# HorizonRobotics/HoloAgent

Measured on AMD Instinct MI355X. Metric: HMSG frames/sec (one scene per GPU: map A1-A2, fusion A3-A5, merge A6, pooling A7, floors A8, rooms by the device watershed N1, room clouds, room embeddings and View nodes A9, objects with the view <-> object test A10 and graph assembly A11, nothing handed in -- plus 1000 coarse-to-fine retrieval qu, higher is better.
Workload: dtype f64 geometry / f32 features

## Files before the change

holoagent_amd/csrc/hmsg_dbscan.h:

```cpp
#pragma once
#include "hmsg_common.h"

#include <vector>

struct PoolSeg {
    long long row_base;
    long long bit_base;
    int n;
    int nw;
    long long tile_base;
    int nt;
    int pad;
};

#define GRAM_T 128

void pool_launch_gram_f32(hipStream_t s, const float* Xn, int D, const PoolSeg* d_ps, int K, long long tiles, float eps, unsigned* adj,
                          unsigned* ncount);
void pool_launch_seg_rows(hipStream_t s, const PoolSeg* d_ps, int K, int maxn, int* seg_of_row);
void pool_cluster(hipStream_t s, const PoolSeg* d_ps, long long R, int minpts, const unsigned* adj, const unsigned* ncount,
                  const int* seg_of_row, int* label, int* seg_first, int* d_changed, int* flabel, unsigned* csize, unsigned* cfirst,
                  unsigned long long* best, DbgLaps* laps = nullptr);
void pool_launch_mean_f32(hipStream_t s, const float* X, int D, const PoolSeg* d_ps, int K, const int* flabel, const unsigned* csize,
                          const unsigned* cfirst, const unsigned long long* best, float* out);

void rn_denoise(hipStream_t s, const void* X, bool f64, int D, const std::vector<long long>& off, double eps, int min_samples, void* out,
                int* n_in_cluster);
void rn_choose(hipStream_t s, const void* rows, bool f64, long long K, int D, const float* T, int n_types, int* d_type);
void rn_vote(hipStream_t s, const int* d_view_type, const std::vector<long long>& voff, int n_types, int* type_of_room );
void rn_gather_rows_f32(hipStream_t s, const float* src, const std::vector<int>& rows, int D, float* dst);
```

holoagent_amd/csrc/hmsg_map.hip:

```cpp
#include "hmsg_common.h"

#include <atomic>

#include <algorithm>


__global__ void k_scan_lookback(const unsigned* __restrict__ in, unsigned* __restrict__ out, size_t n,
                                unsigned long long* __restrict__ state, unsigned epoch) {
    __shared__ unsigned wsum[4];
    __shared__ unsigned s_prefix;
    const int tid = threadIdx.x, lane = tid & 63, w = tid >> 6;
    const long long tile = blockIdx.x;
    const size_t base = ((size_t)tile * 256 + tid) * 4;
    unsigned v[4];
    unsigned t = 0;
    for (int i = 0; i < 4; ++i) {
        v[i] = base + i < n ? in[base + i] : 0u;
        t += v[i];
    }
    unsigned incl = t;
    for (int o = 1; o < 64; o <<= 1) {
        unsigned u = __shfl_up(incl, o);
        if (lane >= o) incl += u;
    }
// ... 133 lines not shown
            atomicMax(&out[3 + a], enc_f64(mx[a]));
        }
        atomicAdd(npts, (unsigned long long)c);
    }
}

__global__ void k_mark(const unsigned short* __restrict__ depth, const double* __restrict__ pose, CamK cam, float scale,
                       int H, int W, int F, GridGeom g, unsigned long long* __restrict__ bitmap) {
    const size_t HW = (size_t)H * W;
    const size_t total = HW * F;
    for (size_t c0 = (size_t)blockIdx.x * PIX_CHUNK; c0 < total; c0 += (size_t)gridDim.x * PIX_CHUNK) {
        const PixWalk pw = pix_walk(c0, HW, W);
        const unsigned npix = (unsigned)(total - c0 < (size_t)PIX_CHUNK ? total - c0 : (size_t)PIX_CHUNK);
        const unsigned fl = pix_last_frame(pw, npix);
        for (unsigned ff = pw.f0; ff <= fl; ++ff) {
            const double* const T = pose + (size_t)ff * 16;
            for (unsigned d = threadIdx.x; d < npix; d += blockDim.x) {
                const size_t i = c0 + d;
                int f, x, y;
                pix_at(pw, d, f, x, y);
                double wx, wy, wz;
                if ((unsigned)f != ff || !backproject(depth[i], x, y, cam, scale, T, wx, wy, wz)) continue;
                int ix, iy, iz;
                cell_of(g, wx, wy, wz, ix, iy, iz);
                long long lin = lin_of(g, ix, iy, iz);
                unsigned long long bit = 1ull << (lin & 63);
                unsigned long long* wp = bitmap + (lin >> 6);
                if (!(*wp & bit)) atomicOr(wp, bit);
            }
        }
    }
}

struct VoxAcc {
    unsigned long long* sr;
    unsigned long long* sg;
    unsigned long long* sb;
    unsigned* n;
};

#define RUN_CHUNK 4096
__device__ __forceinline__ unsigned pixel_slot(const unsigned short* __restrict__ depth, const double* __restrict__ T ,
                                               const CamK& cam, float scale, size_t i, int x, int y, const GridGeom& g,
                                               const unsigned long long* __restrict__ bitmap, const unsigned* __restrict__ rank) {
    double wx, wy, wz;
    if (!backproject(depth[i], x, y, cam, scale, T, wx, wy, wz)) return 0xffffffffu;
    int ix, iy, iz;
    cell_of(g, wx, wy, wz, ix, iy, iz);
    const long long lin = lin_of(g, ix, iy, iz);
    const unsigned long long word = bitmap[lin >> 6];
    return rank[lin >> 6] + (unsigned)__popcll(word & ((1ull << (lin & 63)) - 1ull));
}

__global__ void __launch_bounds__(256) k_slots(const unsigned short* __restrict__ depth, const unsigned char* __restrict__ rgb,
                                               const double* __restrict__ pose, CamK cam, float scale, int H, int W, int F,
                                               GridGeom g, const unsigned long long* __restrict__ bitmap,
                                               const unsigned* __restrict__ rank, VoxAcc acc, unsigned* __restrict__ slots,
                                               unsigned* __restrict__ chunk_runs) {
    __shared__ unsigned s_runs;
    if (threadIdx.x == 0) s_runs = 0u;
    __syncthreads();
    const size_t HW = (size_t)H * W;
    const size_t total = HW * F;
    const int lane = threadIdx.x & 63;
    unsigned myruns = 0;
    const PixWalk pw = pix_walk((size_t)blockIdx.x * RUN_CHUNK, HW, W);
    const size_t left = total - (size_t)blockIdx.x * RUN_CHUNK;
    const unsigned fl = pix_last_frame(pw, (unsigned)(left < (size_t)RUN_CHUNK ? left : (size_t)RUN_CHUNK));
    for (int it = 0; it < RUN_CHUNK / 256; ++it) {
        const size_t i = (size_t)blockIdx.x * RUN_CHUNK + (size_t)it * 256 + threadIdx.x;
        const bool in_range = i < total;
        unsigned slot = 0xffffffffu;
        unsigned cr = 0, cg = 0, cb = 0, cn = 0;
        int x = 0;
        if (in_range) {
            int f, y;
            pix_at(pw, (unsigned)it * 256u + threadIdx.x, f, x, y);
            for (unsigned ff = pw.f0; ff <= fl; ++ff)
                if ((unsigned)f == ff) slot = pixel_slot(depth, pose + (size_t)ff * 16, cam, scale, i, x, y, g, bitmap, rank);
            slots[i] = slot;
            if (slot != 0xffffffffu) {
                const unsigned char* c = rgb + i * 3;
                cr = c[0];
                cg = c[1];
                cb = c[2];
                cn = 1;
            }
        }
        const unsigned prev = __shfl_up(slot, 1);
        int flag = (lane == 0 || prev != slot || x == 0) ? 1 : 0;
        const int head = flag;
        for (int d = 1; d < 64; d <<= 1) {
            unsigned tr = __shfl_up(cr, d), tg = __shfl_up(cg, d), tb = __shfl_up(cb, d), tn = __shfl_up(cn, d);
            int tf = __shfl_up(flag, d);
            if (lane >= d && !flag) {
                cr += tr; cg += tg; cb += tb; cn += tn;
                flag = tf;
            }
        }
        const int nhead = __shfl_down(head, 1);
        const bool tail = lane == 63 || nhead != 0;
        if (tail && slot != 0xffffffffu) {
            atomicAdd(&acc.sr[slot], (unsigned long long)cr);
            atomicAdd(&acc.sg[slot], (unsigned long long)cg);
            atomicAdd(&acc.sb[slot], (unsigned long long)cb);
            atomicAdd(&acc.n[slot], cn);
            ++myruns;
        }
    }
    myruns = (unsigned)wave_sum_i32((int)myruns);
    if (lane == 0 && myruns) atomicAdd(&s_runs, myruns);
    __syncthreads();
    if (threadIdx.x == 0) chunk_runs[blockIdx.x] = s_runs;
}

__global__ void __launch_bounds__(256) k_emit_runs(const unsigned* __restrict__ slots, size_t total, int W, size_t HW,
                                                   const unsigned* __restrict__ chunk_base, unsigned* __restrict__ keys,
                                                   unsigned long long* __restrict__ vals) {
    __shared__ unsigned s_w[4];
    __shared__ unsigned s_run;
    if (threadIdx.x == 0) s_run = chunk_base[blockIdx.x];
    __syncthreads();
    const int lane = threadIdx.x & 63, w = threadIdx.x >> 6;
    const PixWalk pw = pix_walk((size_t)blockIdx.x * RUN_CHUNK, HW, W);
    for (int it = 0; it < RUN_CHUNK / 256; ++it) {
        const size_t i = (size_t)blockIdx.x * RUN_CHUNK + (size_t)it * 256 + threadIdx.x;
        const bool in_range = i < total;
        const unsigned slot = in_range ? slots[i] : 0xffffffffu;
        int pf = 0, x = 0, py = 0;
        if (in_range) pix_at(pw, (unsigned)it * 256u + threadIdx.x, pf, x, py);
        const unsigned prev = __shfl_up(slot, 1);
        const bool head = lane == 0 || prev != slot || x == 0;
        const unsigned long long heads = __ballot(head);
        const int nhead = __shfl_down(head ? 1 : 0, 1);
        const bool tail = (lane == 63 || nhead != 0) && slot != 0xffffffffu;
        const unsigned long long tails = __ballot(tail);
        if (lane == 0) s_w[w] = (unsigned)__popcll(tails);
        __syncthreads();
        unsigned base = s_run;
// ... 77 lines not shown
        }
    }
    if (LDS_SUM) {
        if (lane < 3) pts[v * 3 + lane] = __ddiv_rn(sx, (double)cnt[v]);
    } else if (lane == 0) {
        const double n = (double)cnt[v];
        pts[v * 3 + 0] = __ddiv_rn(sx, n);
        pts[v * 3 + 1] = __ddiv_rn(sy, n);
        pts[v * 3 + 2] = __ddiv_rn(sz, n);
    }
}

__global__ void k_slot_cells(const unsigned long long* __restrict__ bitmap, const unsigned* __restrict__ rank,
                             GridGeom g, int* __restrict__ cell ) {
    long long w = (long long)blockIdx.x * blockDim.x + threadIdx.x;
    if (w >= g.nwords) return;
    unsigned long long bits = bitmap[w];
    unsigned s = rank[w];
    while (bits) {
        int b = __ffsll(bits) - 1;
        bits &= bits - 1;
        long long lin = w * 64 + b;
        int iz = (int)(lin % g.nzp);
        long long r = lin / g.nzp;
        int iy = (int)(r % g.ny);
        int ix = (int)(r / g.ny);
        cell[(size_t)s * 3 + 0] = ix;
        cell[(size_t)s * 3 + 1] = iy;
        cell[(size_t)s * 3 + 2] = iz;
        ++s;
    }
}

__global__ void k_finalize(VoxAcc acc, long long V, double* __restrict__ cols) {
    long long s = (long long)blockIdx.x * blockDim.x + threadIdx.x;
    if (s >= V) return;
    double n = (double)acc.n[s];
    cols[s * 3 + 0] = ((double)acc.sr[s] / 255.0) / n;
    cols[s * 3 + 1] = ((double)acc.sg[s] / 255.0) / n;
    cols[s * 3 + 2] = ((double)acc.sb[s] / 255.0) / n;
}

__device__ __forceinline__ unsigned long long bits_range(int lo, int hi) {
    if (hi < lo) return 0ull;
    unsigned long long m = (hi >= 63) ? ~0ull : ((1ull << (hi + 1)) - 1ull);
    return m & ~((1ull << lo) - 1ull);
}

__global__ void k_outlier(const double* __restrict__ pts, const int* __restrict__ cell, long long V, GridGeom g,
                          const unsigned long long* __restrict__ bitmap, const unsigned* __restrict__ rank,
                          double radius, int nb_points, unsigned* __restrict__ keep) {
    const int lane = threadIdx.x & 63;
    const long long s = ((long long)blockIdx.x * blockDim.x + threadIdx.x) >> 6;
    if (s >= V) return;
    const double px = pts[s * 3], py = pts[s * 3 + 1], pz = pts[s * 3 + 2];
    const int cx = cell[s * 3], cy = cell[s * 3 + 1];
    const int R = (int)ceil(radius / g.vs) + 1;
    const int side = 2 * R + 1;
    const double r2 = radius * radius;
    const double slack = 1e-7;
    int count = 0;
    for (int c = lane; c < side * side; c += 64) {
        int ix = cx - R + c / side, iy = cy - R + c % side;
        if (ix < 0 || iy < 0 || ix >= g.nx || iy >= g.ny) continue;
        double xlo = g.ox + ix * g.vs, xhi = xlo + g.vs, ylo = g.oy + iy * g.vs, yhi = ylo + g.vs;
        double dxmin = fmax(0.0, fmax(xlo - px, px - xhi)), dxmax = fmax(fabs(px - xlo), fabs(px - xhi));
        double dymin = fmax(0.0, fmax(ylo - py, py - yhi)), dymax = fmax(fabs(py - ylo), fabs(py - yhi));
        dxmin = fmax(0.0, dxmin - slack);
        dymin = fmax(0.0, dymin - slack);
        dxmax += slack;
        dymax += slack;
        double rem_out = r2 - (dxmin * dxmin + dymin * dymin);
        if (rem_out <= 0.0) continue;
// ... 9 lines not shown
            if (hi_ > 0.0) {
                zi0 = (int)ceil((pz - hi_ - g.oz) / g.vs);
                zi1 = (int)floor((pz + hi_ - g.oz) / g.vs) - 1;
                zi0 = zi0 < zo0 ? zo0 : zi0;
                zi1 = zi1 > zo1 ? zo1 : zi1;
            }
        }
        long long colw = ((long long)ix * g.ny + iy) * (g.nzp >> 6);
        for (int w = zo0 >> 6; w <= zo1 >> 6; ++w) {
            unsigned long long word = bitmap[colw + w];
            if (!word) continue;
            int b0 = w * 64;
            unsigned long long outer = word & bits_range(zo0 - b0 < 0 ? 0 : zo0 - b0, zo1 - b0 > 63 ? 63 : zo1 - b0);
            unsigned long long inner = 0ull;
            if (zi1 >= zi0) inner = outer & bits_range(zi0 - b0 < 0 ? 0 : zi0 - b0, zi1 - b0 > 63 ? 63 : zi1 - b0);
            count += __popcll(inner);
            unsigned long long shell = outer & ~inner;
            unsigned base = rank[colw + w];
            while (shell) {
                int b = __ffsll(shell) - 1;
                shell &= shell - 1;
                unsigned q = base + (unsigned)__popcll(word & ((1ull << b) - 1ull));
                double dx = pts[(size_t)q * 3] - px, dy = pts[(size_t)q * 3 + 1] - py, dz = pts[(size_t)q * 3 + 2] - pz;
                double d2 = dx * dx + dy * dy + dz * dz;
                count += d2 < r2 ? 1 : 0;
            }
        }
    }
    count = wave_sum_i32(count);
    if (lane == 0) keep[s] = count > nb_points ? 1u : 0u;
}

__global__ void k_compact(const unsigned* __restrict__ keep, const unsigned* __restrict__ newidx, long long V0,
                          const double* __restrict__ pts0, const double* __restrict__ cols0, const int* __restrict__ cell,
                          GridGeom g, double* __restrict__ pts, double* __restrict__ cols,
                          unsigned long long* __restrict__ bitmap) {
    long long s = (long long)blockIdx.x * blockDim.x + threadIdx.x;
    if (s >= V0) return;
    if (keep[s]) {
        unsigned d = newidx[s];
        for (int a = 0; a < 3; ++a) {
            pts[(size_t)d * 3 + a] = pts0[s * 3 + a];
            cols[(size_t)d * 3 + a] = cols0[s * 3 + a];
        }
    } else {
        long long lin = lin_of(g, cell[s * 3], cell[s * 3 + 1], cell[s * 3 + 2]);
        atomicAnd(&bitmap[lin >> 6], ~(1ull << (lin & 63)));
    }
}

__global__ void k_rm_cells(const unsigned* __restrict__ keep, const unsigned* __restrict__ newidx, long long V0,
                           const int* __restrict__ cell, GridGeom g, int* __restrict__ rmcell,
                           unsigned long long* __restrict__ bitmap_rm) {
    long long s = (long long)blockIdx.x * blockDim.x + threadIdx.x;
    if (s >= V0 || keep[s]) return;
    long long r = s - (long long)newidx[s];
    for (int a = 0; a < 3; ++a) rmcell[r * 3 + a] = cell[s * 3 + a];
    long long lin = lin_of(g, cell[s * 3], cell[s * 3 + 1], cell[s * 3 + 2]);
    atomicOr(&bitmap_rm[lin >> 6], 1ull << (lin & 63));
}

template <typename F>
__device__ __forceinline__ void ring_visit(const GridGeom& g, const unsigned long long* __restrict__ bitmap,
                                           const unsigned* __restrict__ rank, int cx, int cy, int cz, int r, int lane, F&& f) {
    const int side = 2 * r + 1;
    for (int ci = lane; ci < side * side; ci += 64) {
        int dx = ci / side - r, dy = ci % side - r;
        int ix = cx + dx, iy = cy + dy;
        if (ix < 0 || iy < 0 || ix >= g.nx || iy >= g.ny) continue;
        bool rim = (dx == -r || dx == r || dy == -r || dy == r);
        long long colw = ((long long)ix * g.ny + iy) * (g.nzp >> 6);
        for (int part = 0; part < (rim ? 1 : 2); ++part) {
            int z0 = rim ? cz - r : (part == 0 ? cz - r : cz + r);
            int z1 = rim ? cz + r : z0;
            z0 = z0 < 0 ? 0 : z0;
            z1 = z1 >= g.nz ? g.nz - 1 : z1;
            if (!rim && (z0 != z1 || (part == 0 ? cz - r < 0 : cz + r >= g.nz))) continue;
// ... 100 lines not shown
                       (const double*)h->pose.p, h->cam, scale, H, W, F, d_b.p, d_b.p + 6);
    HMSG_CHECK_LAUNCH();
    unsigned long long hb[8];
    HIP_TRY(hipMemcpyAsync(hb, d_b.p, sizeof(hb), hipMemcpyDeviceToHost, s));
    HIP_TRY(hipStreamSynchronize(s));
    HMSG_REQUIRE(hb[6] > 0, HMSG_ERR_INVALID, "no valid depth pixel in any frame");
    double mn[3], mx[3];
    for (int a = 0; a < 3; ++a) {
        mn[a] = dec_f64(hb[a]);
        mx[a] = dec_f64(hb[3 + a]);
    }
    GridGeom g;
    g.vs = c.voxel_size;
    g.ox = mn[0] - g.vs * 0.5;
    g.oy = mn[1] - g.vs * 0.5;
    g.oz = mn[2] - g.vs * 0.5;
    g.nx = (int)floor((mx[0] - g.ox) / g.vs) + 2;
    g.ny = (int)floor((mx[1] - g.oy) / g.vs) + 2;
    g.nz = (int)floor((mx[2] - g.oz) / g.vs) + 2;
    g.nzp = (g.nz + 63) / 64 * 64;
    g.nwords = (long long)g.nx * g.ny * (g.nzp / 64);
    HMSG_REQUIRE(g.nwords < (1ll << 31), HMSG_ERR_UNSUPPORTED, "scene bounding box too large for the dense occupancy bitmap");
    h->grid = g;

    h->bitmap.alloc((size_t)g.nwords);
    h->rank.alloc((size_t)g.nwords);
    h->bitmap.zero(s);
    hipLaunchKernelGGL(k_mark, dim3(nblk), dim3(256), 0, s, (const unsigned short*)h->depth.p, (const double*)h->pose.p,
                       h->cam, scale, H, W, F, g, h->bitmap.p);
    HMSG_CHECK_LAUNCH();
    unsigned long long V0 = hmsg_bitmap_rank(h->bitmap.p, h->rank.p, (size_t)g.nwords, s, h->scan_tmp);
    h->V0 = (long long)V0;

    DevBuf<unsigned long long> srgb;
    DevBuf<unsigned> sn, slots, chunk_runs;
    srgb.alloc(V0 * 3);
    sn.alloc(V0);
    srgb.zero(s);
    sn.zero(s);
    slots.alloc(total);
    const unsigned nchunks = cdiv(total, RUN_CHUNK);
    chunk_runs.alloc((size_t)nchunks + 1);
    VoxAcc acc{srgb.p, srgb.p + V0, srgb.p + 2 * V0, sn.p};
    {
        ProfScope ps(h->prof, s, "k_slots", (double)total * 9.0 + (double)V0 * 28.0);
        hipLaunchKernelGGL(k_slots, dim3(nchunks), dim3(256), 0, s, (const unsigned short*)h->depth.p,
                           (const unsigned char*)h->rgb.p, (const double*)h->pose.p, h->cam, scale, H, W, F, g,
                           (const unsigned long long*)h->bitmap.p, (const unsigned*)h->rank.p, acc, slots.p, chunk_runs.p);
    }
    HMSG_CHECK_LAUNCH();
    unsigned long long nruns = 0;
    hmsg_scan_u32(chunk_runs.p, chunk_runs.p, (size_t)nchunks, s, h->scan_tmp, &nruns);
    SortBufs sb;
    sb.keys.alloc((size_t)std::max<unsigned long long>(nruns, 1));
    sb.vals.alloc((size_t)std::max<unsigned long long>(nruns, 1));
    HMSG_REQUIRE(W < 4096 && H < 4096, HMSG_ERR_UNSUPPORTED, "image sides must be below 4096 pixels");
    hipLaunchKernelGGL(k_emit_runs, dim3(nchunks), dim3(256), 0, s, (const unsigned*)slots.p, total, W, (size_t)H * W,
                       (const unsigned*)chunk_runs.p, sb.keys.p, sb.vals.p);
    HMSG_CHECK_LAUNCH();
    {
        ProfScope ps(h->prof, s, "sort_runs", (double)nruns * 12.0 * 4.0);
        hmsg_sort_pairs(sb, (size_t)nruns, bits_for(V0), s);
    }
    DevBuf<unsigned> run_off;
    run_off.alloc(V0 + 1);
    hmsg_sort_segment_starts(sb.res_keys, (size_t)nruns, run_off.p, (unsigned)V0, s);
    DevBuf<int> cell;
    cell.alloc(V0 * 3);
    hipLaunchKernelGGL(k_slot_cells, dim3(cdiv((size_t)g.nwords, 256)), dim3(256), 0, s,
                       (const unsigned long long*)h->bitmap.p, (const unsigned*)h->rank.p, g, cell.p);
    HMSG_CHECK_LAUNCH();
    DevBuf<double> pts0, cols0;
    pts0.alloc(V0 * 3);
    cols0.alloc(V0 * 3);
    {
        static const bool lds_sum = getenv("HMSG_DEBUG_ACCUM_WAVES") == nullptr;
        ProfScope ps(h->prof, s, "k_accum_ordered", (double)total * 2.0 + (double)nruns * 8.0 + (double)V0 * 32.0);
        hipLaunchKernelGGL(lds_sum ? k_accum_ordered<true> : k_accum_ordered<false>, dim3(cdiv(V0 * 64, 256)), dim3(256), 0, s,
                           (const unsigned short*)h->depth.p, (const double*)h->pose.p, h->cam, scale, W, (size_t)H * W, (long long)V0,
                           (const unsigned*)run_off.p, (const unsigned long long*)sb.res_vals, (const unsigned*)sn.p, pts0.p);
        HMSG_CHECK_LAUNCH();
        if (getenv("HMSG_DEBUG_ACCUM_STATS")) {
            std::vector<unsigned> hc((size_t)V0);
            HIP_TRY(hipMemcpyAsync(hc.data(), sn.p, (size_t)V0 * 4, hipMemcpyDeviceToHost, s));
            HIP_TRY(hipStreamSynchronize(s));
            std::sort(hc.begin(), hc.end());
            double tot = 0;
            for (unsigned c : hc) tot += c;
            fprintf(stderr, "[hmsg map] voxels %lld  runs %llu  pixels %.0f  max %u  median %u  p99 %u\n", (long long)V0, nruns, tot, hc.back(),
                    hc[hc.size() / 2], hc[(size_t)(hc.size() * 0.99)]);
            for (unsigned th : {512u, 2048u, 8192u, 32768u, 131072u}) {
                double px = 0;
                long long nv = 0;
                for (unsigned c : hc)
                    if (c > th) px += c, ++nv;
                fprintf(stderr, "[hmsg map]   more than %6u pixels: %7lld voxels holding %.3f of the pixels\n", th, nv, px / tot);
            }
        }
    }
    hipLaunchKernelGGL(k_finalize, dim3(cdiv(V0, 256)), dim3(256), 0, s, acc, (long long)V0, cols0.p);
    HMSG_CHECK_LAUNCH();

    DevBuf<unsigned> keep, newidx;
    keep.alloc(V0);
    newidx.alloc(V0);
    hipLaunchKernelGGL(k_outlier, dim3(cdiv(V0 * 64, 256)), dim3(256), 0, s, (const double*)pts0.p, (const int*)cell.p,
                       (long long)V0, g, (const unsigned long long*)h->bitmap.p, (const unsigned*)h->rank.p,
                       c.outlier_radius, c.outlier_nb_points, keep.p);
    HMSG_CHECK_LAUNCH();
    unsigned long long V = 0;
    hmsg_scan_u32(keep.p, newidx.p, V0, s, h->scan_tmp, &V);
    h->V = (long long)V;
    h->pts.alloc(V * 3);
    h->cols.alloc(V * 3);
    hipLaunchKernelGGL(k_compact, dim3(cdiv(V0, 256)), dim3(256), 0, s, (const unsigned*)keep.p, (const unsigned*)newidx.p,
                       (long long)V0, (const double*)pts0.p, (const double*)cols0.p, (const int*)cell.p, g, h->pts.p,
                       h->cols.p, h->bitmap.p);
    HMSG_CHECK_LAUNCH();
    unsigned long long V2 = hmsg_bitmap_rank(h->bitmap.p, h->rank.p, (size_t)g.nwords, s, h->scan_tmp);
    HMSG_REQUIRE(V2 == V, HMSG_ERR_INVALID, "internal: filtered bitmap population mismatch");
    const long long VR = (long long)V0 - (long long)V;
    h->have_cand = false;
    if (VR > 0 && V > 0) {
        h->bitmap_rm.alloc((size_t)g.nwords);
        h->rank_rm.alloc((size_t)g.nwords);
        h->bitmap_rm.zero(s);
        DevBuf<int> rmcell, rend;
        DevBuf<double> ub2;
        DevBuf<unsigned> ccnt, cursor;
        rmcell.alloc((size_t)VR * 3);
        rend.alloc((size_t)VR);
        ub2.alloc((size_t)VR);
        ccnt.alloc((size_t)VR + 1);
        cursor.alloc((size_t)VR);
        ccnt.zero(s);
        cursor.zero(s);
        hipLaunchKernelGGL(k_rm_cells, dim3(cdiv(V0, 256)), dim3(256), 0, s, (const unsigned*)keep.p, (const unsigned*)newidx.p,
                           (long long)V0, (const int*)cell.p, g, rmcell.p, h->bitmap_rm.p);
        HMSG_CHECK_LAUNCH();
        unsigned long long nrm = hmsg_bitmap_rank(h->bitmap_rm.p, h->rank_rm.p, (size_t)g.nwords, s, h->scan_tmp);
        HMSG_REQUIRE((long long)nrm == VR, HMSG_ERR_INVALID, "internal: removed-cell bitmap population mismatch");
        h->cand_off.alloc((size_t)VR + 1);
        {
            ProfScope ps(h->prof, s, "k_cand");
            hipLaunchKernelGGL(k_cand, dim3(cdiv((size_t)VR * 64, 256)), dim3(256), 0, s, 0, (const int*)rmcell.p, VR, g,
                               (const unsigned long long*)h->bitmap.p, (const unsigned*)h->rank.p, (const double*)h->pts.p, ub2.p,
                               rend.p, ccnt.p, (const unsigned*)nullptr, (int*)nullptr, (unsigned*)nullptr);
        }
        HMSG_CHECK_LAUNCH();
        unsigned long long ncand = 0;
// ... 13 lines not shown
```

holoagent_amd/csrc/hmsg_pool.hip:

```cpp
#include "hmsg_boundary.h"
#include "hmsg_cloudops.h"
#include "hmsg_nn.h"
#include "hmsg_dbscan.h"

#include <algorithm>
#include <cmath>

typedef float f32x16 __attribute__((ext_vector_type(16)));

__global__ void k_pool_nn(const double* __restrict__ q, long long N, NNIndex I, double max_dist, int* __restrict__ idx,
                          unsigned* __restrict__ valid, TieList ties) {
    long long i = (long long)blockIdx.x * blockDim.x + threadIdx.x;
    if (i >= N) return;
    double d2 = 0;
    int ntie = 0;
    int v = nn_search(I, q[i * 3], q[i * 3 + 1], q[i * 3 + 2], &d2, &ntie);
    if (ntie > 1) tie_push(ties, i, q[i * 3], q[i * 3 + 1], q[i * 3 + 2]);
    idx[i] = v;
    valid[i] = (v >= 0 && __dsqrt_rn(d2) <= max_dist) ? 1u : 0u;
}

__global__ void k_pool_gather(const int* __restrict__ idx, const unsigned* __restrict__ valid, const unsigned* __restrict__ pos,
                              long long N, const float* __restrict__ feats, int D, float* __restrict__ X, float* __restrict__ Xn) {
    const int lane = threadIdx.x & 63;
    const long long i = ((long long)blockIdx.x * blockDim.x + threadIdx.x) >> 6;
    if (i >= N || !valid[i]) return;
    const float* src = feats + (size_t)idx[i] * D;
    float* dx = X + (size_t)pos[i] * D;
    float* dn = Xn + (size_t)pos[i] * D;
    float n2 = 0.f;
    for (int e = lane; e < D; e += 64) {
        float v = src[e];
        if (v != v) v = 0.f;
        else if (v > 3.4028234663852886e38f) v = 3.4028234663852886e38f;
        else if (v < -3.4028234663852886e38f) v = -3.4028234663852886e38f;
        dx[e] = v;
        n2 += v * v;
    }
    float nrm = __fsqrt_rn(wave_sum_f32(n2));
    if (nrm == 0.f) nrm = 1.f;
    for (int e = lane; e < D; e += 64) dn[e] = __fdiv_rn(dx[e], nrm);
}

#define GRAM_SUP 8
__device__ __forceinline__ void gram_tile_of(long long t, int nt, int& ti, int& tj) {
    int I = 0, r0 = 0, hgt = 0;
    for (;;) {
        r0 = I * GRAM_SUP;
        hgt = min(nt, r0 + GRAM_SUP) - r0;
        const long long cnt = (long long)hgt * (nt - r0) - (long long)hgt * (hgt - 1) / 2;
        if (t < cnt) break;
        t -= cnt;
        ++I;
    }
    const long long dcnt = (long long)hgt * (hgt + 1) / 2;
    if (t < dcnt) {
        int r = 0, len = hgt;
        while (t >= len) {
            t -= len;
            --len;
            ++r;
        }
        ti = r0 + r;
        tj = ti + (int)t;
        return;
    }
    t -= dcnt;
    for (int J = I + 1;; ++J) {
        const int w = min(GRAM_SUP, nt - J * GRAM_SUP);
        const long long c = (long long)hgt * w;
        if (t < c) {
            ti = r0 + (int)(t / w);
            tj = J * GRAM_SUP + (int)(t % w);
            return;
// ... 196 lines not shown
        const unsigned* row = adj + sg.bit_base + (size_t)(i - sg.row_base) * sg.nw;
        for (int w = lane; w < sg.nw; w += 64) {
            unsigned bits = row[w];
            while (bits) {
                int b = __ffs(bits) - 1;
                bits &= bits - 1;
                long long j = sg.row_base + (long long)w * 32 + b;
                if (ncount[j] >= (unsigned)minpts) best = label[j] < best ? label[j] : best;
            }
        }
        for (int o = 32; o > 0; o >>= 1) {
            int t = __shfl_xor(best, o);
            best = t < best ? t : best;
        }
        if (best == 0x7fffffff) best = -1;
    }
    if (lane == 0) {
        final_label[i] = best;
        if (best >= 0) {
            atomicAdd(&csize[sg.row_base + best], 1u);
            atomicMin(&cfirst[sg.row_base + best], (unsigned)(i - sg.row_base));
        }
    }
}
__global__ void k_pool_pick(const PoolSeg* __restrict__ segs, const int* __restrict__ seg_of_row, long long N,
                            const unsigned* __restrict__ csize, const unsigned* __restrict__ cfirst,
                            unsigned long long* __restrict__ best) {
    long long i = (long long)blockIdx.x * blockDim.x + threadIdx.x;
    if (i >= N || csize[i] == 0u) return;
    unsigned long long key = ((unsigned long long)csize[i] << 32) | (unsigned long long)(0xffffffffu - cfirst[i]);
    atomicMax(&best[seg_of_row[i]], key);
}
#define POOL_MEAN_AHEAD 16
__global__ void k_pool_mean(const float* __restrict__ X, int D, const PoolSeg* __restrict__ segs, int K,
                            const int* __restrict__ final_label, const unsigned* __restrict__ csize,
                            const unsigned* __restrict__ cfirst, const unsigned long long* __restrict__ best,
                            float* __restrict__ out) {
    const int k = blockIdx.y;
    const int d = blockIdx.x * blockDim.x + threadIdx.x;
    if (d >= D) return;
    const PoolSeg sg = segs[k];
    float* o = out + (size_t)k * D;
    if (sg.n == 0) {
        o[d] = 0.f;
        return;
    }
    int want = -2;
    unsigned long long key = best[k];
    if (key) {
        unsigned first = 0xffffffffu - (unsigned)(key & 0xffffffffull);
        want = final_label[sg.row_base + first];
    }
    float acc = 0.f;
    unsigned cnt = 0;
    const float* const xb = X + (size_t)sg.row_base * D + d;
    const int* const lb = final_label + sg.row_base;
    float cur[POOL_MEAN_AHEAD], nxt[POOL_MEAN_AHEAD];
    int curl[POOL_MEAN_AHEAD], nxtl[POOL_MEAN_AHEAD];
#pragma unroll
    for (int j = 0; j < POOL_MEAN_AHEAD; ++j) {
        const int rr = min(j, sg.n - 1);
        cur[j] = xb[(size_t)rr * D];
        curl[j] = lb[rr];
    }
    for (int r = 0; r < sg.n; r += POOL_MEAN_AHEAD) {
        if (r + POOL_MEAN_AHEAD < sg.n) {
#pragma unroll
            for (int j = 0; j < POOL_MEAN_AHEAD; ++j) {
                const int rr = min(r + POOL_MEAN_AHEAD + j, sg.n - 1);
                nxt[j] = xb[(size_t)rr * D];
                nxtl[j] = lb[rr];
            }
        }
#pragma unroll
        for (int j = 0; j < POOL_MEAN_AHEAD; ++j) {
            if (r + j < sg.n && (want == -2 || curl[j] == want)) {
                acc = __fadd_rn(acc, cur[j]);
                ++cnt;
            }
        }
#pragma unroll
        for (int j = 0; j < POOL_MEAN_AHEAD; ++j) {
            cur[j] = nxt[j];
            curl[j] = nxtl[j];
        }
    }
    o[d] = cnt > 1 ? __fdiv_rn(acc, (float)cnt) : acc;
}

__global__ void k_pool_gather_u32(const unsigned* __restrict__ src, const long long* __restrict__ idx, int n,
                                  unsigned* __restrict__ dst) {
    int t = blockIdx.x * blockDim.x + threadIdx.x;
    if (t < n) dst[t] = src[idx[t]];
}
__global__ void k_seg_rows(const PoolSeg* __restrict__ segs, int* __restrict__ seg_of_row) {
    const PoolSeg sg = segs[blockIdx.y];
    for (int i = blockIdx.x * blockDim.x + threadIdx.x; i < sg.n; i += gridDim.x * blockDim.x) seg_of_row[sg.row_base + i] = blockIdx.y;
}

void pool_cluster(hipStream_t s, const PoolSeg* d_ps, long long R, int minpts, const unsigned* adj, const unsigned* ncount,
                  const int* seg_of_row, int* label, int* seg_first, int* d_changed, int* flabel, unsigned* csize, unsigned* cfirst,
                  unsigned long long* best, DbgLaps* laps) {
    hipLaunchKernelGGL(k_pool_init, dim3(cdiv((size_t)R, 256)), dim3(256), 0, s, ncount, (long long)R,
                       minpts, label, d_ps, seg_of_row, seg_first);
    HMSG_CHECK_LAUNCH();
    DevBuf<unsigned> open_list;
    open_list.alloc((size_t)std::max<long long>(R, 1) + 1);
    const unsigned* d_list = nullptr;
    unsigned n_open = 0;
    static const bool list_wanted = getenv("HMSG_DEBUG_POOL_ALL_ROWS") == nullptr;
    for (int it = 0; it < 100000; ++it) {
        HIP_TRY(hipMemsetAsync(d_changed, 0, 4, s));
        const size_t rows = d_list ? (size_t)n_open : (size_t)R;
        for (int rep = 0; rep < (it == 0 ? 2 : 1) && rows; ++rep) {
            hipLaunchKernelGGL(k_pool_prop, dim3(cdiv(rows * 64, 256)), dim3(256), 0, s, adj,
                               d_ps, seg_of_row, ncount,
                               minpts, (long long)rows, label, d_changed, seg_first, (it == 0 && rep == 0) ? 1 : 0, d_list);
// ... 5 lines not shown
            HIP_TRY(hipMemsetAsync(open_list.p, 0, 4, s));
            hipLaunchKernelGGL(k_pool_list, dim3(cdiv((size_t)R, 256)), dim3(256), 0, s, d_ps, seg_of_row,
                               ncount, minpts, (long long)R, label, seg_first,
                               open_list.p + 1, open_list.p);
            HMSG_CHECK_LAUNCH();
            HIP_TRY(hipMemcpyAsync(&n_open, open_list.p, 4, hipMemcpyDeviceToHost, s));
        }
        int ch = 0;
        HIP_TRY(hipMemcpyAsync(&ch, d_changed, 4, hipMemcpyDeviceToHost, s));
        HIP_TRY(hipStreamSynchronize(s));
        if (it == 0 && list_wanted) d_list = open_list.p + 1;
        if (!ch) break;
    }
    if (laps) laps->lap("label propagation");
    hipLaunchKernelGGL(k_pool_border, dim3(cdiv((size_t)R * 64, 256)), dim3(256), 0, s, adj,
                       d_ps, seg_of_row, ncount, minpts,
                       (long long)R, label, flabel, csize, cfirst);
    hipLaunchKernelGGL(k_pool_pick, dim3(cdiv((size_t)R, 256)), dim3(256), 0, s, d_ps,
                       seg_of_row, (long long)R, csize, cfirst, best);
    HMSG_CHECK_LAUNCH();
}

void pool_launch_gram_f32(hipStream_t s, const float* Xn, int D, const PoolSeg* d_ps, int K, long long tiles, float eps, unsigned* adj,
                          unsigned* ncount) {
    hipLaunchKernelGGL(k_pool_gram, dim3((unsigned)tiles), dim3(256), 0, s, Xn, D, d_ps, K, eps, adj, ncount);
    HMSG_CHECK_LAUNCH();
}
void pool_launch_seg_rows(hipStream_t s, const PoolSeg* d_ps, int K, int maxn, int* seg_of_row) {
    hipLaunchKernelGGL(k_seg_rows, dim3(std::max(1u, std::min(cdiv(maxn, 256), 256u)), K), dim3(256), 0, s, d_ps, seg_of_row);
    HMSG_CHECK_LAUNCH();
}
void pool_launch_mean_f32(hipStream_t s, const float* X, int D, const PoolSeg* d_ps, int K, const int* flabel, const unsigned* csize,
                          const unsigned* cfirst, const unsigned long long* best, float* out) {
    hipLaunchKernelGGL(k_pool_mean, dim3(cdiv(D, 64), K), dim3(64), 0, s, X, D, d_ps, K, flabel, csize, cfirst, best, out);
    HMSG_CHECK_LAUNCH();
}

static void pool_rows(hipStream_t s, DevBuf<unsigned>& scan_tmp, Prof* prof, DbgLaps& laps, const int* idx, const unsigned* valid,
                      long long P, const std::vector<int>& dn, const float* feats, int D, double eps, int minpts, float* out) {
    const int K = (int)dn.size();
    DevBuf<unsigned> pos;
    pos.alloc((size_t)std::max<long long>(P, 1));
    unsigned long long R = 0;
    if (P) hmsg_scan_u32(valid, pos.p, (size_t)P, s, scan_tmp, &R);
    std::vector<long long> pstart(K + 1, 0);
    for (int k = 0; k < K; ++k) pstart[k + 1] = pstart[k] + dn[k];
    std::vector<unsigned> hpos(K + 1, (unsigned)R);
    {
        DevBuf<long long> d_i;
        DevBuf<unsigned> d_o;
        std::vector<long long> q;
        std::vector<int> which;
        for (int k = 0; k < K; ++k)
            if (pstart[k] < P) {
                q.push_back(pstart[k]);
                which.push_back(k);
            }
        if (!q.empty()) {
            std::vector<unsigned> tmp(q.size());
            d_i.alloc(q.size());
            d_o.alloc(q.size());
            HIP_TRY(hipMemcpyAsync(d_i.p, q.data(), q.size() * 8, hipMemcpyHostToDevice, s));
            hipLaunchKernelGGL(k_pool_gather_u32, dim3(cdiv(q.size(), 256)), dim3(256), 0, s, (const unsigned*)pos.p,
                               (const long long*)d_i.p, (int)q.size(), d_o.p);
            HIP_TRY(hipMemcpyAsync(tmp.data(), d_o.p, q.size() * 4, hipMemcpyDeviceToHost, s));
            HIP_TRY(hipStreamSynchronize(s));
            for (size_t t = 0; t < q.size(); ++t) hpos[which[t]] = tmp[t];
        }
        for (int k = K - 1; k >= 0; --k)
            if (pstart[k] >= P) hpos[k] = hpos[k + 1];
    }
    std::vector<PoolSeg> ps(K);
    long long bitw = 0, tiles = 0;
    int maxn = 0;
    for (int k = 0; k < K; ++k) {
        PoolSeg& g = ps[k];
        g.row_base = hpos[k];
        g.n = (int)(hpos[k + 1] - hpos[k]);
        g.nw = (g.n + 31) / 32;
        g.nt = (g.n + GRAM_T - 1) / GRAM_T;
        g.bit_base = bitw;
        g.tile_base = tiles;
        g.pad = 0;
        bitw += (long long)g.n * g.nw;
        tiles += (long long)g.nt * (g.nt + 1) / 2;
        maxn = std::max(maxn, g.n);
    }
    DevBuf<PoolSeg> d_ps;
    d_ps.alloc(K);
    HIP_TRY(hipMemcpyAsync(d_ps.p, ps.data(), (size_t)K * sizeof(PoolSeg), hipMemcpyHostToDevice, s));
    DevBuf<float> X, Xn;
    DevBuf<unsigned> adj, ncount, csize, cfirst;
    DevBuf<int> label, flabel, seg_of_row, d_changed, seg_first;
    DevBuf<unsigned long long> best;
    const size_t Rn = (size_t)std::max<unsigned long long>(R, 1);
    X.alloc(Rn * D);
    Xn.alloc(Rn * D);
    adj.alloc((size_t)std::max<long long>(bitw, 1));
    ncount.alloc(Rn);
    csize.alloc(Rn);
    cfirst.alloc(Rn);
    label.alloc(Rn);
    flabel.alloc(Rn);
    seg_of_row.alloc(Rn);
    d_changed.alloc(1);
    seg_first.alloc((size_t)std::max(K, 1));
    HIP_TRY(hipMemsetAsync(seg_first.p, 0x7f, (size_t)std::max(K, 1) * 4, s));
    best.alloc(K);
    adj.zero(s);
    ncount.zero(s);
    csize.zero(s);
    HIP_TRY(hipMemsetAsync(cfirst.p, 0xff, Rn * 4, s));
    best.zero(s);
    laps.lap("row offsets + buffers");
    if (R) {
        hipLaunchKernelGGL(k_pool_gather, dim3(cdiv((size_t)P * 64, 256)), dim3(256), 0, s, idx,
                           valid, (const unsigned*)pos.p, P, feats, D, X.p, Xn.p);
        hipLaunchKernelGGL(k_seg_rows, dim3(std::max(1u, std::min(cdiv(maxn, 256), 256u)), K), dim3(256), 0, s,
                           (const PoolSeg*)d_ps.p, seg_of_row.p);
        laps.lap("gather + normalise");
        {
            double flop = 0;
            for (auto& g : ps) flop += (double)g.n * ((double)g.n + 1.0) * D;
            ProfScope psc(prof, s, "k_pool_gram", flop);
            hipLaunchKernelGGL(k_pool_gram, dim3((unsigned)tiles), dim3(256), 0, s, (const float*)Xn.p, D, (const PoolSeg*)d_ps.p, K,
                               (float)eps, adj.p, ncount.p);
        }
        laps.lap("k_pool_gram");
        pool_cluster(s, (const PoolSeg*)d_ps.p, (long long)R, minpts, (const unsigned*)adj.p, (const unsigned*)ncount.p,
                     (const int*)seg_of_row.p, label.p, seg_first.p, d_changed.p, flabel.p, csize.p, cfirst.p, best.p, &laps);
    }
    laps.lap("border + pick");
    hmsg_dump("pool_ncount", ncount.p, (size_t)R * 4, s);
    hmsg_dump("pool_flabel", flabel.p, (size_t)R * 4, s);
    hmsg_dump("pool_label", label.p, (size_t)R * 4, s);
    hmsg_dump("pool_segs", d_ps.p, (size_t)K * sizeof(PoolSeg), s);
    hipLaunchKernelGGL(k_pool_mean, dim3(cdiv(D, 64), K), dim3(64), 0, s, (const float*)X.p, D, (const PoolSeg*)d_ps.p, K,
                       (const int*)flabel.p, (const unsigned*)csize.p, (const unsigned*)cfirst.p,
                       (const unsigned long long*)best.p, out);
    HMSG_CHECK_LAUNCH();
    HIP_TRY(hipStreamSynchronize(s));
    laps.lap("k_pool_mean");
}

void hmsg_pool(hmsg_ctx* h) {
    const hmsg_config& c = h->cfg;
    hipStream_t s = h->stream;
    HMSG_REQUIRE(h->merged, HMSG_ERR_INVALID, "hmsg_pool_instances: run hmsg_merge_instances first");
    const int K = (int)h->inst.off.size() - 1;
    const int D = c.feat_dim;
    h->inst_feats.alloc((size_t)std::max(K, 1) * D);
    if (K == 0) {
        h->pooled = true;
        return;
    }
    CloudOps ops;
    ops.s = s;
    DbgLaps laps("pool", s);
    std::vector<SegDesc> segs(K);
    for (int k = 0; k < K; ++k) {
        segs[k].pt_base = h->inst.off[k];
        segs[k].n = (int)(h->inst.off[k + 1] - h->inst.off[k]);
    }
    ops.bounds(h->inst.pts.p, segs);
    DevBuf<double> ds;
    ds.alloc((size_t)std::max<long long>(h->inst.total, 1) * 3);
    std::vector<int> dn;
    const long long P = ops.voxel_down_sample(h->inst.pts.p, segs, c.voxel_size, ds.p, dn);
    laps.lap("voxel_down_sample");
    DevBuf<int> idx;
    DevBuf<unsigned> valid;
    idx.alloc((size_t)std::max<long long>(P, 1));
    valid.alloc((size_t)std::max<long long>(P, 1));
// ... 61 lines not shown
```

Measured before the change: 2639.

## Defer voxel colour sums to kept voxels and gather pooled features by index

Voxel colour accumulation no longer does three 64-bit atomics per run in k_slots. Colours are now computed only for kept voxels after compaction, by walking the sorted run records and reading RGB again. The pooling stage drops the dense X copy of features and stores only a source-row index. The mean kernel then gathers from the original feature table, with nan_to_num applied on the fly and a deeper prefetch of labels and indices. This cuts atomics, buffer traffic and one full feature copy, in exchange for scattered gather reads and a second pass over RGB.

Result: faster. 2683, median of 4 (+1.7%).

```diff
diff --git a/holoagent_amd/csrc/hmsg_dbscan.h b/holoagent_amd/csrc/hmsg_dbscan.h
--- a/holoagent_amd/csrc/hmsg_dbscan.h
+++ b/holoagent_amd/csrc/hmsg_dbscan.h
@@ -23,6 +23,8 @@
                   unsigned long long* best, DbgLaps* laps = nullptr);
 void pool_launch_mean_f32(hipStream_t s, const float* X, int D, const PoolSeg* d_ps, int K, const int* flabel, const unsigned* csize,
                           const unsigned* cfirst, const unsigned long long* best, float* out);
+void pool_launch_mean_gather_f32(hipStream_t s, const float* table, const int* src_row, int D, const PoolSeg* d_ps, int K, const int* flabel,
+                                 const unsigned* csize, const unsigned* cfirst, const unsigned long long* best, float* out);
 
 void rn_denoise(hipStream_t s, const void* X, bool f64, int D, const std::vector<long long>& off, double eps, int min_samples, void* out,
                 int* n_in_cluster);
diff --git a/holoagent_amd/csrc/hmsg_map.hip b/holoagent_amd/csrc/hmsg_map.hip
--- a/holoagent_amd/csrc/hmsg_map.hip
+++ b/holoagent_amd/csrc/hmsg_map.hip
@@ -189,13 +189,6 @@
     }
 }
 
-struct VoxAcc {
-    unsigned long long* sr;
-    unsigned long long* sg;
-    unsigned long long* sb;
-    unsigned* n;
-};
-
 #define RUN_CHUNK 4096
 __device__ __forceinline__ unsigned pixel_slot(const unsigned short* __restrict__ depth, const double* __restrict__ T ,
                                                const CamK& cam, float scale, size_t i, int x, int y, const GridGeom& g,
@@ -209,11 +202,10 @@
     return rank[lin >> 6] + (unsigned)__popcll(word & ((1ull << (lin & 63)) - 1ull));
 }
 
-__global__ void __launch_bounds__(256) k_slots(const unsigned short* __restrict__ depth, const unsigned char* __restrict__ rgb,
-                                               const double* __restrict__ pose, CamK cam, float scale, int H, int W, int F,
+__global__ void __launch_bounds__(256) k_slots(const unsigned short* __restrict__ depth, const double* __restrict__ pose, CamK cam, float scale, int H, int W, int F,
                                                GridGeom g, const unsigned long long* __restrict__ bitmap,
-                                               const unsigned* __restrict__ rank, VoxAcc acc, unsigned* __restrict__ slots,
-                                               unsigned* __restrict__ chunk_runs) {
+                                               const unsigned* __restrict__ rank, unsigned* __restrict__ vox_n,
+                                               unsigned* __restrict__ slots, unsigned* __restrict__ chunk_runs) {
     __shared__ unsigned s_runs;
     if (threadIdx.x == 0) s_runs = 0u;
     __syncthreads();
@@ -228,7 +220,7 @@
         const size_t i = (size_t)blockIdx.x * RUN_CHUNK + (size_t)it * 256 + threadIdx.x;
         const bool in_range = i < total;
         unsigned slot = 0xffffffffu;
-        unsigned cr = 0, cg = 0, cb = 0, cn = 0;
+        unsigned cn = 0;
         int x = 0;
         if (in_range) {
             int f, y;
@@ -236,32 +228,23 @@
             for (unsigned ff = pw.f0; ff <= fl; ++ff)
                 if ((unsigned)f == ff) slot = pixel_slot(depth, pose + (size_t)ff * 16, cam, scale, i, x, y, g, bitmap, rank);
             slots[i] = slot;
-            if (slot != 0xffffffffu) {
-                const unsigned char* c = rgb + i * 3;
-                cr = c[0];
-                cg = c[1];
-                cb = c[2];
-                cn = 1;
-            }
+            if (slot != 0xffffffffu) cn = 1;
         }
         const unsigned prev = __shfl_up(slot, 1);
         int flag = (lane == 0 || prev != slot || x == 0) ? 1 : 0;
         const int head = flag;
         for (int d = 1; d < 64; d <<= 1) {
-            unsigned tr = __shfl_up(cr, d), tg = __shfl_up(cg, d), tb = __shfl_up(cb, d), tn = __shfl_up(cn, d);
+            unsigned tn = __shfl_up(cn, d);
             int tf = __shfl_up(flag, d);
             if (lane >= d && !flag) {
-                cr += tr; cg += tg; cb += tb; cn += tn;
+                cn += tn;
                 flag = tf;
             }
         }
         const int nhead = __shfl_down(head, 1);
         const bool tail = lane == 63 || nhead != 0;
         if (tail && slot != 0xffffffffu) {
-            atomicAdd(&acc.sr[slot], (unsigned long long)cr);
-            atomicAdd(&acc.sg[slot], (unsigned long long)cg);
-            atomicAdd(&acc.sb[slot], (unsigned long long)cb);
-            atomicAdd(&acc.n[slot], cn);
+            atomicAdd(&vox_n[slot], cn);
             ++myruns;
         }
     }
@@ -405,13 +388,42 @@
     }
 }
 
-__global__ void k_finalize(VoxAcc acc, long long V, double* __restrict__ cols) {
-    long long s = (long long)blockIdx.x * blockDim.x + threadIdx.x;
-    if (s >= V) return;
-    double n = (double)acc.n[s];
-    cols[s * 3 + 0] = ((double)acc.sr[s] / 255.0) / n;
-    cols[s * 3 + 1] = ((double)acc.sg[s] / 255.0) / n;
-    cols[s * 3 + 2] = ((double)acc.sb[s] / 255.0) / n;
+__global__ void __launch_bounds__(256) k_colours_kept(const unsigned char* __restrict__ rgb, int W, size_t HW, long long V0,
+                                                      const unsigned* __restrict__ keep, const unsigned* __restrict__ newidx,
+                                                      const unsigned* __restrict__ off, const unsigned long long* __restrict__ runs,
+                                                      const unsigned* __restrict__ cnt, double* __restrict__ cols) {
+    const int lane = threadIdx.x & 63;
+    const long long v = ((long long)blockIdx.x * blockDim.x + threadIdx.x) >> 6;
+    if (v >= V0 || !keep[v]) return;
+    unsigned long long sr = 0ull, sg = 0ull, sb = 0ull;
+    const unsigned r1 = off[v + 1];
+    for (unsigned r = off[v] + lane; r < r1; r += 64) {
+        const unsigned long long rec = runs[r];
+        const int len = (int)(rec & 255ull);
+        const size_t f = (size_t)(rec >> 32), y = (size_t)((rec >> 20) & 0xfffull), x0 = (size_t)((rec >> 8) & 0xfffull);
+        const unsigned char* c = rgb + (f * HW + y * (size_t)W + x0) * 3;
+        unsigned pr = 0, pg = 0, pb = 0;
+        for (int j = 0; j < len; ++j) {
+            pr += c[j * 3];
+            pg += c[j * 3 + 1];
+            pb += c[j * 3 + 2];
+        }
+        sr += pr;
+        sg += pg;
+        sb += pb;
+    }
+    for (int o = 32; o > 0; o >>= 1) {
+        sr += __shfl_xor(sr, o);
+        sg += __shfl_xor(sg, o);
+        sb += __shfl_xor(sb, o);
+    }
+    if (lane == 0) {
+        const double n = (double)cnt[v];
+        double* o = cols + (size_t)newidx[v] * 3;
+        o[0] = ((double)sr / 255.0) / n;
+        o[1] = ((double)sg / 255.0) / n;
+        o[2] = ((double)sb / 255.0) / n;
+    }
 }
 
 __device__ __forceinline__ unsigned long long bits_range(int lo, int hi) {
@@ -487,17 +499,13 @@
 }
 
 __global__ void k_compact(const unsigned* __restrict__ keep, const unsigned* __restrict__ newidx, long long V0,
-                          const double* __restrict__ pts0, const double* __restrict__ cols0, const int* __restrict__ cell,
-                          GridGeom g, double* __restrict__ pts, double* __restrict__ cols,
+                          const double* __restrict__ pts0, const int* __restrict__ cell, GridGeom g, double* __restrict__ pts,
                           unsigned long long* __restrict__ bitmap) {
     long long s = (long long)blockIdx.x * blockDim.x + threadIdx.x;
     if (s >= V0) return;
     if (keep[s]) {
         unsigned d = newidx[s];
-        for (int a = 0; a < 3; ++a) {
-            pts[(size_t)d * 3 + a] = pts0[s * 3 + a];
-            cols[(size_t)d * 3 + a] = cols0[s * 3 + a];
-        }
+        for (int a = 0; a < 3; ++a) pts[(size_t)d * 3 + a] = pts0[s * 3 + a];
     } else {
         long long lin = lin_of(g, cell[s * 3], cell[s * 3 + 1], cell[s * 3 + 2]);
         atomicAnd(&bitmap[lin >> 6], ~(1ull << (lin & 63)));
@@ -664,21 +672,17 @@
     unsigned long long V0 = hmsg_bitmap_rank(h->bitmap.p, h->rank.p, (size_t)g.nwords, s, h->scan_tmp);
     h->V0 = (long long)V0;
 
-    DevBuf<unsigned long long> srgb;
     DevBuf<unsigned> sn, slots, chunk_runs;
-    srgb.alloc(V0 * 3);
     sn.alloc(V0);
-    srgb.zero(s);
     sn.zero(s);
     slots.alloc(total);
     const unsigned nchunks = cdiv(total, RUN_CHUNK);
     chunk_runs.alloc((size_t)nchunks + 1);
-    VoxAcc acc{srgb.p, srgb.p + V0, srgb.p + 2 * V0, sn.p};
     {
-        ProfScope ps(h->prof, s, "k_slots", (double)total * 9.0 + (double)V0 * 28.0);
-        hipLaunchKernelGGL(k_slots, dim3(nchunks), dim3(256), 0, s, (const unsigned short*)h->depth.p,
-                           (const unsigned char*)h->rgb.p, (const double*)h->pose.p, h->cam, scale, H, W, F, g,
-                           (const unsigned long long*)h->bitmap.p, (const unsigned*)h->rank.p, acc, slots.p, chunk_runs.p);
+        ProfScope ps(h->prof, s, "k_slots", (double)total * 6.0 + (double)V0 * 4.0);
+        hipLaunchKernelGGL(k_slots, dim3(nchunks), dim3(256), 0, s, (const unsigned short*)h->depth.p, (const double*)h->pose.p, h->cam,
+                           scale, H, W, F, g, (const unsigned long long*)h->bitmap.p, (const unsigned*)h->rank.p, sn.p, slots.p,
+                           chunk_runs.p);
     }
     HMSG_CHECK_LAUNCH();
     unsigned long long nruns = 0;
@@ -702,9 +706,8 @@
     hipLaunchKernelGGL(k_slot_cells, dim3(cdiv((size_t)g.nwords, 256)), dim3(256), 0, s,
                        (const unsigned long long*)h->bitmap.p, (const unsigned*)h->rank.p, g, cell.p);
     HMSG_CHECK_LAUNCH();
-    DevBuf<double> pts0, cols0;
+    DevBuf<double> pts0;
     pts0.alloc(V0 * 3);
-    cols0.alloc(V0 * 3);
     {
         static const bool lds_sum = getenv("HMSG_DEBUG_ACCUM_WAVES") == nullptr;
         ProfScope ps(h->prof, s, "k_accum_ordered", (double)total * 2.0 + (double)nruns * 8.0 + (double)V0 * 32.0);
@@ -730,8 +733,6 @@
             }
         }
     }
-    hipLaunchKernelGGL(k_finalize, dim3(cdiv(V0, 256)), dim3(256), 0, s, acc, (long long)V0, cols0.p);
-    HMSG_CHECK_LAUNCH();
 
     DevBuf<unsigned> keep, newidx;
     keep.alloc(V0);
@@ -746,8 +747,14 @@
     h->pts.alloc(V * 3);
     h->cols.alloc(V * 3);
     hipLaunchKernelGGL(k_compact, dim3(cdiv(V0, 256)), dim3(256), 0, s, (const unsigned*)keep.p, (const unsigned*)newidx.p,
-                       (long long)V0, (const double*)pts0.p, (const double*)cols0.p, (const int*)cell.p, g, h->pts.p,
-                       h->cols.p, h->bitmap.p);
+                       (long long)V0, (const double*)pts0.p, (const int*)cell.p, g, h->pts.p, h->bitmap.p);
+    HMSG_CHECK_LAUNCH();
+    {
+        ProfScope ps(h->prof, s, "k_colours_kept");
+        hipLaunchKernelGGL(k_colours_kept, dim3(cdiv(V0 * 64, 256)), dim3(256), 0, s, (const unsigned char*)h->rgb.p, W, (size_t)H * W,
+                           (long long)V0, (const unsigned*)keep.p, (const unsigned*)newidx.p, (const unsigned*)run_off.p,
+                           (const unsigned long long*)sb.res_vals, (const unsigned*)sn.p, h->cols.p);
+    }
     HMSG_CHECK_LAUNCH();
     unsigned long long V2 = hmsg_bitmap_rank(h->bitmap.p, h->rank.p, (size_t)g.nwords, s, h->scan_tmp);
     HMSG_REQUIRE(V2 == V, HMSG_ERR_INVALID, "internal: filtered bitmap population mismatch");
diff --git a/holoagent_amd/csrc/hmsg_pool.hip b/holoagent_amd/csrc/hmsg_pool.hip
--- a/holoagent_amd/csrc/hmsg_pool.hip
+++ b/holoagent_amd/csrc/hmsg_pool.hip
@@ -20,26 +20,28 @@
     valid[i] = (v >= 0 && __dsqrt_rn(d2) <= max_dist) ? 1u : 0u;
 }
 
+__device__ __forceinline__ float pool_nan_to_num(float v) {
+    if (v != v) return 0.f;
+    if (v > 3.4028234663852886e38f) return 3.4028234663852886e38f;
+    if (v < -3.4028234663852886e38f) return -3.4028234663852886e38f;
+    return v;
+}
 __global__ void k_pool_gather(const int* __restrict__ idx, const unsigned* __restrict__ valid, const unsigned* __restrict__ pos,
-                              long long N, const float* __restrict__ feats, int D, float* __restrict__ X, float* __restrict__ Xn) {
+                              long long N, const float* __restrict__ feats, int D, int* __restrict__ src_row, float* __restrict__ Xn) {
     const int lane = threadIdx.x & 63;
     const long long i = ((long long)blockIdx.x * blockDim.x + threadIdx.x) >> 6;
     if (i >= N || !valid[i]) return;
     const float* src = feats + (size_t)idx[i] * D;
-    float* dx = X + (size_t)pos[i] * D;
     float* dn = Xn + (size_t)pos[i] * D;
+    if (lane == 0) src_row[pos[i]] = idx[i];
     float n2 = 0.f;
     for (int e = lane; e < D; e += 64) {
-        float v = src[e];
-        if (v != v) v = 0.f;
-        else if (v > 3.4028234663852886e38f) v = 3.4028234663852886e38f;
-        else if (v < -3.4028234663852886e38f) v = -3.4028234663852886e38f;
-        dx[e] = v;
+        const float v = pool_nan_to_num(src[e]);
         n2 += v * v;
     }
     float nrm = __fsqrt_rn(wave_sum_f32(n2));
     if (nrm == 0.f) nrm = 1.f;
-    for (int e = lane; e < D; e += 64) dn[e] = __fdiv_rn(dx[e], nrm);
+    for (int e = lane; e < D; e += 64) dn[e] = __fdiv_rn(pool_nan_to_num(src[e]), nrm);
 }
 
 #define GRAM_SUP 8
@@ -302,7 +304,8 @@
     atomicMax(&best[seg_of_row[i]], key);
 }
 #define POOL_MEAN_AHEAD 16
-__global__ void k_pool_mean(const float* __restrict__ X, int D, const PoolSeg* __restrict__ segs, int K,
+template <bool GATHER>
+__global__ void k_pool_mean(const float* __restrict__ X, const int* __restrict__ src_row, int D, const PoolSeg* __restrict__ segs, int K,
                             const int* __restrict__ final_label, const unsigned* __restrict__ csize,
                             const unsigned* __restrict__ cfirst, const unsigned long long* __restrict__ best,
                             float* __restrict__ out) {
@@ -323,23 +326,52 @@
     }
     float acc = 0.f;
     unsigned cnt = 0;
-    const float* const xb = X + (size_t)sg.row_base * D + d;
+    const float* const xb = GATHER ? X + d : X + (size_t)sg.row_base * D + d;
     const int* const lb = final_label + sg.row_base;
+    const int* const sb = GATHER ? src_row + sg.row_base : nullptr;
     float cur[POOL_MEAN_AHEAD], nxt[POOL_MEAN_AHEAD];
     int curl[POOL_MEAN_AHEAD], nxtl[POOL_MEAN_AHEAD];
+    int nxts[POOL_MEAN_AHEAD], farl[POOL_MEAN_AHEAD], fars[POOL_MEAN_AHEAD];
+    if (GATHER) {
 #pragma unroll
-    for (int j = 0; j < POOL_MEAN_AHEAD; ++j) {
-        const int rr = min(j, sg.n - 1);
-        cur[j] = xb[(size_t)rr * D];
-        curl[j] = lb[rr];
+        for (int j = 0; j < POOL_MEAN_AHEAD; ++j) {
+            const int r0 = min(j, sg.n - 1), r1 = min(POOL_MEAN_AHEAD + j, sg.n - 1);
+            curl[j] = lb[r0];
+            nxts[j] = sb[r0];
+            farl[j] = lb[r1];
+            fars[j] = sb[r1];
+        }
+#pragma unroll
+        for (int j = 0; j < POOL_MEAN_AHEAD; ++j) {
+            cur[j] = (want == -2 || curl[j] == want) ? pool_nan_to_num(xb[(size_t)nxts[j] * D]) : 0.f;
+            nxtl[j] = farl[j];
+            nxts[j] = fars[j];
+        }
+    } else {
+#pragma unroll
+        for (int j = 0; j < POOL_MEAN_AHEAD; ++j) {
+            const int rr = min(j, sg.n - 1);
+            cur[j] = xb[(size_t)rr * D];
+            curl[j] = lb[rr];
+        }
     }
     for (int r = 0; r < sg.n; r += POOL_MEAN_AHEAD) {
         if (r + POOL_MEAN_AHEAD < sg.n) {
+            if (GATHER) {
 #pragma unroll
-            for (int j = 0; j < POOL_MEAN_AHEAD; ++j) {
-                const int rr = min(r + POOL_MEAN_AHEAD + j, sg.n - 1);
-                nxt[j] = xb[(size_t)rr * D];
-                nxtl[j] = lb[rr];
+                for (int j = 0; j < POOL_MEAN_AHEAD; ++j) {
+                    nxt[j] = (want == -2 || nxtl[j] == want) ? pool_nan_to_num(xb[(size_t)nxts[j] * D]) : 0.f;
+                    const int rr = min(r + 2 * POOL_MEAN_AHEAD + j, sg.n - 1);
+                    farl[j] = lb[rr];
+                    fars[j] = sb[rr];
+                }
+            } else {
+#pragma unroll
+                for (int j = 0; j < POOL_MEAN_AHEAD; ++j) {
+                    const int rr = min(r + POOL_MEAN_AHEAD + j, sg.n - 1);
+                    nxt[j] = xb[(size_t)rr * D];
+                    nxtl[j] = lb[rr];
+                }
             }
         }
 #pragma unroll
@@ -353,6 +385,10 @@
         for (int j = 0; j < POOL_MEAN_AHEAD; ++j) {
             cur[j] = nxt[j];
             curl[j] = nxtl[j];
+            if (GATHER) {
+                nxtl[j] = farl[j];
+                nxts[j] = fars[j];
+            }
         }
     }
     o[d] = cnt > 1 ? __fdiv_rn(acc, (float)cnt) : acc;
@@ -424,7 +460,13 @@
 }
 void pool_launch_mean_f32(hipStream_t s, const float* X, int D, const PoolSeg* d_ps, int K, const int* flabel, const unsigned* csize,
                           const unsigned* cfirst, const unsigned long long* best, float* out) {
-    hipLaunchKernelGGL(k_pool_mean, dim3(cdiv(D, 64), K), dim3(64), 0, s, X, D, d_ps, K, flabel, csize, cfirst, best, out);
+    hipLaunchKernelGGL(k_pool_mean<false>, dim3(cdiv(D, 64), K), dim3(64), 0, s, X, (const int*)nullptr, D, d_ps, K, flabel, csize, cfirst, best,
+                       out);
+    HMSG_CHECK_LAUNCH();
+}
+void pool_launch_mean_gather_f32(hipStream_t s, const float* table, const int* src_row, int D, const PoolSeg* d_ps, int K, const int* flabel,
+                                 const unsigned* csize, const unsigned* cfirst, const unsigned long long* best, float* out) {
+    hipLaunchKernelGGL(k_pool_mean<true>, dim3(cdiv(D, 64), K), dim3(64), 0, s, table, src_row, D, d_ps, K, flabel, csize, cfirst, best, out);
     HMSG_CHECK_LAUNCH();
 }
 
@@ -481,12 +523,13 @@
     DevBuf<PoolSeg> d_ps;
     d_ps.alloc(K);
     HIP_TRY(hipMemcpyAsync(d_ps.p, ps.data(), (size_t)K * sizeof(PoolSeg), hipMemcpyHostToDevice, s));
-    DevBuf<float> X, Xn;
+    DevBuf<float> Xn;
+    DevBuf<int> src_row;
     DevBuf<unsigned> adj, ncount, csize, cfirst;
     DevBuf<int> label, flabel, seg_of_row, d_changed, seg_first;
     DevBuf<unsigned long long> best;
     const size_t Rn = (size_t)std::max<unsigned long long>(R, 1);
-    X.alloc(Rn * D);
+    src_row.alloc(Rn);
     Xn.alloc(Rn * D);
     adj.alloc((size_t)std::max<long long>(bitw, 1));
     ncount.alloc(Rn);
@@ -507,7 +550,7 @@
     laps.lap("row offsets + buffers");
     if (R) {
         hipLaunchKernelGGL(k_pool_gather, dim3(cdiv((size_t)P * 64, 256)), dim3(256), 0, s, idx,
-                           valid, (const unsigned*)pos.p, P, feats, D, X.p, Xn.p);
+                           valid, (const unsigned*)pos.p, P, feats, D, src_row.p, Xn.p);
         hipLaunchKernelGGL(k_seg_rows, dim3(std::max(1u, std::min(cdiv(maxn, 256), 256u)), K), dim3(256), 0, s,
                            (const PoolSeg*)d_ps.p, seg_of_row.p);
         laps.lap("gather + normalise");
@@ -527,10 +570,8 @@
     hmsg_dump("pool_flabel", flabel.p, (size_t)R * 4, s);
     hmsg_dump("pool_label", label.p, (size_t)R * 4, s);
     hmsg_dump("pool_segs", d_ps.p, (size_t)K * sizeof(PoolSeg), s);
-    hipLaunchKernelGGL(k_pool_mean, dim3(cdiv(D, 64), K), dim3(64), 0, s, (const float*)X.p, D, (const PoolSeg*)d_ps.p, K,
-                       (const int*)flabel.p, (const unsigned*)csize.p, (const unsigned*)cfirst.p,
-                       (const unsigned long long*)best.p, out);
-    HMSG_CHECK_LAUNCH();
+    pool_launch_mean_gather_f32(s, feats, (const int*)src_row.p, D, (const PoolSeg*)d_ps.p, K, (const int*)flabel.p, (const unsigned*)csize.p,
+                                (const unsigned*)cfirst.p, (const unsigned long long*)best.p, out);
     HIP_TRY(hipStreamSynchronize(s));
     laps.lap("k_pool_mean");
 }
```
